# linnanwang/FastGen

Measured on AMD Instinct MI355X. Metric: images/sec at 4-step distilled (DMD2) sampling, higher is better.
Workload: dtype fp32 (tensors, accumulate) with split-bf16 x3 MFMA conv products; 1 GPU; EDM CIFAR-10 32x32 SongUNet (55.7M params) DMD2 4-step 'sde' sampling, batch=512 per GPU; global_batch=512, sample_steps=4, parallelism=replicas x1 (no data-path collective), graph=True

## Files before the change

fastgen_amd/csrc/attn.hip:

```cpp
#include <cstdlib>
#include "common.h"
#include "misc.h"

namespace {

template <typename T>
struct PFrag;
template <>
struct PFrag<__bf16> {
    static __device__ __forceinline__ Frag8<__bf16> make(const f32x16& p, int s) {
        Frag8<__bf16> f;
#pragma unroll
        for (int j = 0; j < 8; ++j) f.v[j] = (__bf16)p[8 * s + j];
        return f;
    }
};
template <>
struct PFrag<float> {
    static __device__ __forceinline__ Frag8<float> make(const f32x16& p, int s) {
        Frag8<float> f;
        f.lo = f32x4{p[8 * s + 0], p[8 * s + 1], p[8 * s + 2], p[8 * s + 3]};
        f.hi = f32x4{p[8 * s + 4], p[8 * s + 5], p[8 * s + 6], p[8 * s + 7]};
        return f;
    }
// ... 216 lines not shown
            sum += e;
        }
    sum += __shfl_xor(sum, 32);
    const float inv = __builtin_amdgcn_rcpf(sum);
    Frag8<__bf16> pf[8][2];
#pragma unroll
    for (int kt = 0; kt < 8; ++kt) {
#pragma unroll
        for (int s2 = 0; s2 < 2; ++s2)
#pragma unroll
            for (int j = 0; j < 8; ++j) pf[kt][s2].v[j] = (__bf16)(st[kt][8 * s2 + j] * inv);
        __builtin_amdgcn_sched_barrier(0);
    }

    __builtin_amdgcn_sched_barrier(0);
    __bf16* obase = out + ((size_t)n * Tn + q0) * D + r;
#pragma unroll 1
    for (int dg = 0; dg < 2; ++dg) {
        f32x16 o[4];
#pragma unroll
        for (int d = 0; d < 4; ++d)
#pragma unroll
            for (int i = 0; i < 16; ++i) o[d][i] = 0.f;
        asm volatile("" ::: "memory");
        stage_v(0, smem);
        __syncthreads();
#pragma unroll
        for (int t = 0; t < 4; ++t) {
            const char* cur = smem + (t & 1) * ATT_BUF;
            if (t + 1 < 4) stage_v(t + 1, smem + ((t + 1) & 1) * ATT_BUF);
#pragma unroll
            for (int sub = 0; sub < 2; ++sub)
#pragma unroll
                for (int s2 = 0; s2 < 2; ++s2)
#pragma unroll
                    for (int d = 0; d < 4; ++d) {
                        const char* p = cur + ((dg * 4 + d) * 32 + r) * VPITCH + (sub * 32 + 16 * s2 + 4 * h) * 2;
                        const bf16x4 lo = *reinterpret_cast<const bf16x4*>(p);
                        const bf16x4 hi = *reinterpret_cast<const bf16x4*>(p + 16);
                        Frag8<__bf16> vf;
                        vf.v = bf16x8{lo[0], lo[1], lo[2], lo[3], hi[0], hi[1], hi[2], hi[3]};
                        mma16(o[d], pf[t * 2 + sub][s2], vf);
                    }
            __syncthreads();
            __builtin_amdgcn_sched_barrier(0);
        }
#pragma unroll
        for (int d = 0; d < 4; ++d)
#pragma unroll
            for (int i = 0; i < 16; ++i) obase[(size_t)acc_row(i, h) * D + (dg * 4 + d) * 32] = (__bf16)o[d][i];
    }
}

constexpr int X3_KP = 272, X3_VP = 136;
constexpr int X3_PLANE = 64 * X3_KP;
constexpr int X3_BUF = 2 * X3_PLANE;

struct AttnMerge {
    const float2* ab;
    const float* bp;
    float2* stats;
    float scale;
};

template <bool MRG>
__global__ __launch_bounds__(256, 2) void attention_x3_lds_kernel(const float* __restrict__ q, const float* __restrict__ k,
                                                                  const float* __restrict__ vt, float* __restrict__ out, int B,
                                                                  AttnMerge mg) {
    constexpr int Tn = 256, D = 256;
    extern __shared__ __attribute__((aligned(16))) char smem[];
    const int tid = threadIdx.x, lane = tid & 63, wave = tid >> 6;
    const int r = lane & 31, h = lane >> 5;
    const int n = blockIdx.x >> 1;
    const int q0 = (blockIdx.x & 1) * 128 + wave * 32;

    auto stage_k = [&](int s, char* buf) {
        const float* src = k + ((size_t)n * Tn + (s & 3) * 64) * D + (s >> 2) * 128;
        f32x4 cf[4];
        if constexpr (MRG) {
            const f32x4* cp = reinterpret_cast<const f32x4*>(mg.ab + (size_t)n * D + (s >> 2) * 128 + (tid & 15) * 8);
#pragma unroll
            for (int j = 0; j < 4; ++j) cf[j] = cp[j];
        }
#pragma unroll
        for (int b2 = 0; b2 < 2; ++b2) {
#pragma unroll
            for (int i = b2 * 2; i < b2 * 2 + 2; ++i) {
                const int idx = tid + 256 * i, row = idx >> 4, c = idx & 15;
                float x[8];
                widen8(load_frag(src + (size_t)row * D + c * 8), x);
                if constexpr (MRG) {
#pragma unroll
                    for (int j = 0; j < 8; ++j) x[j] = fmaf(x[j], cf[j >> 1][2 * (j & 1)], cf[j >> 1][2 * (j & 1) + 1]);
                }
                bf16x8 hi, lo;
                split8(x, hi, lo);
                *reinterpret_cast<bf16x8*>(buf + row * X3_KP + c * 16) = hi;
                *reinterpret_cast<bf16x8*>(buf + X3_PLANE + row * X3_KP + c * 16) = lo;
            }
            __builtin_amdgcn_sched_barrier(0);
        }
    };
    auto stage_v = [&](int s, char* buf) {
        const float* src = vt + ((size_t)n * D + (s >> 2) * 128) * Tn + (s & 3) * 64;
#pragma unroll
        for (int b2 = 0; b2 < 2; ++b2) {
#pragma unroll
            for (int i = b2 * 2; i < b2 * 2 + 2; ++i) {
                const int idx = tid + 256 * i, row = idx >> 3, c = idx & 7;
                float x[8];
                widen8(load_frag(src + (size_t)row * Tn + c * 8), x);
                bf16x8 hi, lo;
                split8(x, hi, lo);
                bf16x4* dh = reinterpret_cast<bf16x4*>(buf + row * X3_VP + c * 16);
                dh[0] = bf16x4{hi[0], hi[1], hi[2], hi[3]};
                dh[1] = bf16x4{hi[4], hi[5], hi[6], hi[7]};
                bf16x4* dl = reinterpret_cast<bf16x4*>(buf + X3_PLANE + row * X3_VP + c * 16);
                dl[0] = bf16x4{lo[0], lo[1], lo[2], lo[3]};
                dl[1] = bf16x4{lo[4], lo[5], lo[6], lo[7]};
            }
            __builtin_amdgcn_sched_barrier(0);
        }
    };

    const float* qrow = q + ((size_t)n * Tn + q0 + r) * D + 8 * h;
    f32x16 st[8];
#pragma unroll
    for (int kt = 0; kt < 8; ++kt)
#pragma unroll
        for (int i = 0; i < 16; ++i) st[kt][i] = 0.f;

    stage_k(0, smem);
    __syncthreads();
    Frag8<bf16x3> qf[8];
#pragma unroll
    for (int s = 0; s < 8; ++s) {
        const char* cur = smem + (s & 1) * X3_BUF;
        if ((s & 3) == 0) {
#pragma unroll
            for (int kk = 0; kk < 8; ++kk) qf[kk] = load_op<bf16x3>(qrow + (s >> 2) * 128 + kk * 16);
        }
        if (s + 1 < 8) stage_k(s + 1, smem + ((s + 1) & 1) * X3_BUF);
#pragma unroll
        for (int kk = 0; kk < 8; ++kk) {
#pragma unroll
            for (int sub = 0; sub < 2; ++sub) {
                const char* p = cur + (sub * 32 + r) * X3_KP + (kk * 16 + 8 * h) * 2;
                Frag8<bf16x3> kf;
                kf.hi = *reinterpret_cast<const bf16x8*>(p);
                kf.lo = *reinterpret_cast<const bf16x8*>(p + X3_PLANE);
                mma16(st[(s & 3) * 2 + sub], kf, qf[kk]);
            }
        }
        __syncthreads();
        __builtin_amdgcn_sched_barrier(0);
    }

    float m = -INFINITY;
#pragma unroll
    for (int kt = 0; kt < 8; ++kt)
#pragma unroll
        for (int i = 0; i < 16; ++i) m = fmaxf(m, st[kt][i]);
    m = fmaxf(m, __shfl_xor(m, 32));
    float sum = 0.f;
#pragma unroll
    for (int kt = 0; kt < 8; ++kt)
#pragma unroll
        for (int i = 0; i < 16; ++i) {
            const float e = __builtin_amdgcn_exp2f(1.44269504088896341f * 0.0625f * (st[kt][i] - m));
            st[kt][i] = e;
            sum += e;
        }
    sum += __shfl_xor(sum, 32);
    const float inv = __builtin_amdgcn_rcpf(sum);
    Frag8<bf16x3> pf[8][2];
#pragma unroll
    for (int kt = 0; kt < 8; ++kt) {
#pragma unroll
        for (int s2 = 0; s2 < 2; ++s2) {
            float v[8];
#pragma unroll
            for (int j = 0; j < 8; ++j) v[j] = st[kt][8 * s2 + j] * inv;
            split8(v, pf[kt][s2].hi, pf[kt][s2].lo);
        }
        __builtin_amdgcn_sched_barrier(0);
    }

    float* obase = out + ((size_t)n * Tn + q0) * D + r;
    stage_v(0, smem);
    __syncthreads();
    f32x16 o[4];
#pragma unroll
    for (int s = 0; s < 8; ++s) {
        const char* cur = smem + (s & 1) * X3_BUF;
        if ((s & 3) == 0) {
#pragma unroll
            for (int d = 0; d < 4; ++d)
#pragma unroll
                for (int i = 0; i < 16; ++i) o[d][i] = 0.f;
        }
        if (s + 1 < 8) stage_v(s + 1, smem + ((s + 1) & 1) * X3_BUF);
#pragma unroll
        for (int sub = 0; sub < 2; ++sub)
#pragma unroll
            for (int s2 = 0; s2 < 2; ++s2)
#pragma unroll
                for (int d = 0; d < 4; ++d) {
                    const char* p = cur + (d * 32 + r) * X3_VP + (sub * 32 + 16 * s2 + 4 * h) * 2;
                    const bf16x4 a0 = *reinterpret_cast<const bf16x4*>(p), a1 = *reinterpret_cast<const bf16x4*>(p + 16);
                    const bf16x4 b0 = *reinterpret_cast<const bf16x4*>(p + X3_PLANE), b1 = *reinterpret_cast<const bf16x4*>(p + X3_PLANE + 16);
                    Frag8<bf16x3> vf;
                    vf.hi = bf16x8{a0[0], a0[1], a0[2], a0[3], a1[0], a1[1], a1[2], a1[3]};
                    vf.lo = bf16x8{b0[0], b0[1], b0[2], b0[3], b1[0], b1[1], b1[2], b1[3]};
                    mma16(o[d], pf[(s & 3) * 2 + sub][s2], vf);
                }
        __syncthreads();
        __builtin_amdgcn_sched_barrier(0);
        if ((s & 3) == 3) {
            if constexpr (MRG) {
                const float* xbase = k + ((size_t)n * Tn + q0) * D + r;
#pragma unroll
                for (int d = 0; d < 4; ++d) {
                    const int col = ((s >> 2) * 4 + d) * 32;
                    const float bias = mg.bp[col + r];
                    float sv = 0.f, qv = 0.f;
#pragma unroll
                    for (int i = 0; i < 16; ++i) {
                        const size_t off = (size_t)acc_row(i, h) * D + col;
                        const float v = (o[d][i] + bias + xbase[off]) * mg.scale;
                        obase[off] = v;
                        sv += v;
                        qv += v * v;
                    }
                    if (mg.stats) {
                        sv += __shfl_xor(sv, 32), qv += __shfl_xor(qv, 32);
                        sv += __shfl_xor(sv, 1), qv += __shfl_xor(qv, 1);
                        sv += __shfl_xor(sv, 2), qv += __shfl_xor(qv, 2);
                        if (h == 0 && (r & 3) == 0)
                            mg.stats[((size_t)n * 8 + (blockIdx.x & 1) * 4 + wave) * (D / 4) + ((col + r) >> 2)] = make_float2(sv, qv);
                    }
                }
            } else {
#pragma unroll
                for (int d = 0; d < 4; ++d)
#pragma unroll
                    for (int i = 0; i < 16; ++i) obase[(size_t)acc_row(i, h) * D + ((s >> 2) * 4 + d) * 32] = o[d][i];
            }
        }
    }
}

__global__ void attn_merge_weights_kernel(const float* __restrict__ qkv_w, const float* __restrict__ qkv_b, const float* __restrict__ proj_w,
                                          float* __restrict__ w_out, float* __restrict__ b_out, int C) {
    const int o = blockIdx.x % C;
    const bool val = blockIdx.x >= C;
    for (int i = threadIdx.x; i <= C; i += blockDim.x) {
        double acc = 0.0;
        for (int c = 0; c < C; ++c) {
            const double l = val ? proj_w[(size_t)o * C + c] : qkv_w[(size_t)(3 * c + 1) * C + o];
            const int row = 3 * c + (val ? 2 : 0);
            acc += l * (double)(i < C ? qkv_w[(size_t)row * C + i] : qkv_b[row]);
        }
        if (i < C)
            w_out[(size_t)blockIdx.x * C + i] = (float)acc;
        else
            b_out[blockIdx.x] = (float)acc;
    }
}

template <bool MRG>
int x3_lds_prepare() {
    static bool done[16] = {};
    const int dev = fg_device_slot();
    if (dev < 0) return (int)hipErrorInvalidDevice;
    if (!done[dev]) {
        hipError_t e = hipFuncSetAttribute(reinterpret_cast<const void*>(attention_x3_lds_kernel<MRG>), hipFuncAttributeMaxDynamicSharedMemorySize, 2 * X3_BUF);
        if (e != hipSuccess) return (int)e;
        done[dev] = true;
    }
    return 0;
}

}

int launch_attn_merge_weights(const float* qkv_w, const float* qkv_b, const float* proj_w, float* w_out, float* b_out, int C, hipStream_t s) {
    hipLaunchKernelGGL(attn_merge_weights_kernel, dim3(2 * C), dim3(256), 0, s, qkv_w, qkv_b, proj_w, w_out, b_out, C);
    return (int)hipGetLastError();
}

int launch_attention_merged(const float* qm, const float* x_mid, const float2* ab, const float* vmt, const float* bp, float scale, float* out,
                            float2* stats, int B, hipStream_t s) {
    const int rc = x3_lds_prepare<true>();
    if (rc || !qm) return rc;
    hipLaunchKernelGGL(attention_x3_lds_kernel<true>, dim3(B * 2), dim3(256), 2 * X3_BUF, s, qm, x_mid, vmt, out, B, AttnMerge{ab, bp, stats, scale});
    return (int)hipGetLastError();
}

int launch_attention(int dtype, const void* q, const void* k, const void* vt, void* out, int B, int T, hipStream_t s) {
    if (T != 256 && T != 64) return (int)hipErrorInvalidValue;
    const int nt = T / 32;
    const int waves = B * nt;
    dim3 grid((waves + 3) / 4), block(256);
    if (dtype == 1 && nt == 8) {
        static bool attr_done_dev[16] = {};
        const int dev = fg_device_slot();
        if (dev < 0) return (int)hipErrorInvalidDevice;
        bool& attr_done = attr_done_dev[dev];
        if (!attr_done) {
            hipError_t e = hipFuncSetAttribute(reinterpret_cast<const void*>(attention_lds_kernel), hipFuncAttributeMaxDynamicSharedMemorySize, 2 * ATT_BUF);
            if (e != hipSuccess) return (int)e;
            attr_done = true;
        }
        if (!q) return 0;
        hipLaunchKernelGGL(attention_lds_kernel, dim3(B * 2), block, 2 * ATT_BUF, s, (const __bf16*)q, (const __bf16*)k, (const __bf16*)vt, (__bf16*)out, B);
        return (int)hipGetLastError();
    }
    static const bool x3_lds = [] {
        const char* e = getenv("FASTGEN_AMD_ATTN_X3_LDS");
        return !(e && e[0] == '0');
    }();
    if (dtype == 2 && nt == 8 && x3_lds) {
        const int rc = x3_lds_prepare<false>();
        if (rc || !q) return rc;
        hipLaunchKernelGGL(attention_x3_lds_kernel<false>, dim3(B * 2), block, 2 * X3_BUF, s, (const float*)q, (const float*)k, (const float*)vt, (float*)out, B,
                           AttnMerge{});
        return (int)hipGetLastError();
    }
    if (!q) return 0;
    if (dtype == 2) {
        if (nt == 8)
            hipLaunchKernelGGL((attention_kernel<bf16x3, 8>), grid, block, 0, s, (const float*)q, (const float*)k, (const float*)vt, (float*)out, B);
        else
            hipLaunchKernelGGL((attention_kernel<bf16x3, 2>), grid, block, 0, s, (const float*)q, (const float*)k, (const float*)vt, (float*)out, B);
    } else if (dtype) {
        if (nt == 8)
            hipLaunchKernelGGL((attention_kernel<__bf16, 8>), grid, block, 0, s, (const __bf16*)q, (const __bf16*)k, (const __bf16*)vt, (__bf16*)out, B);
        else
            hipLaunchKernelGGL((attention_kernel<__bf16, 2>), grid, block, 0, s, (const __bf16*)q, (const __bf16*)k, (const __bf16*)vt, (__bf16*)out, B);
    } else {
        if (nt == 8)
            hipLaunchKernelGGL((attention_kernel<float, 8>), grid, block, 0, s, (const float*)q, (const float*)k, (const float*)vt, (float*)out, B);
        else
            hipLaunchKernelGGL((attention_kernel<float, 2>), grid, block, 0, s, (const float*)q, (const float*)k, (const float*)vt, (float*)out, B);
    }
    return (int)hipGetLastError();
}
```

fastgen_amd/csrc/engine.hip:

```cpp
#include <hip/hip_runtime.h>

#include <atomic>
#include <cmath>
#include <cstdarg>
#include <cstdio>
#include <cstdlib>
#include <cstring>
#include <string>
#include <map>
#include <vector>

#include "../../include/fastgen_amd.h"
#include "common.h"
#include "adm.h"
#include "edm2.h"
#include "conv.h"
#include "misc.h"

namespace {

thread_local std::string g_err;

int fail(int code, const char* fmt, ...) {
    char buf[512];
// ... 695 lines not shown
void use_stash(Workspace& w, const BlockStash& st) {
    w.h.p = st.h;
    w.ab0 = st.ab0, w.ab1 = st.ab1, w.mr0 = st.mr0, w.mr1 = st.mr1;
    w.a1d = st.a1d;
    w.drop.block = st.index;
    if (st.xattn) {
        w.xattn.p = st.xattn;
        w.ab2 = st.ab2, w.mr2 = st.mr2;
        w.q = st.q, w.k = st.k, w.vt = st.vt, w.aout = st.aout;
    }
}
int block_index(const fg_edm* h, const Block* b) {
    for (size_t i = 0; i < h->blocks.size(); ++i)
        if (h->blocks[i] == b) return (int)i;
    return -1;
}

bool attn_merge_enabled() {
    static const bool on = [] {
        const char* e = getenv("FASTGEN_AMD_ATTN_MERGE");
        return !(e && e[0] == '0');
    }();
    return on;
}

int run_block(fg_edm* h, const Block& b, const Act& x1, int c1, const Act& x2, int c2, const float* temb, Act& out, int B,
              Workspace& w, hipStream_t s) {
    if (c1 + c2 != b.cin) return fail(FG_EINVAL, "%s: got %d+%d input channels, expected %d", b.key.c_str(), c1, c2, b.cin);
    const int hw_in = b.res_in * b.res_in, hw = b.res_out * b.res_out;
    const int res_mode = b.down ? RES_DOWN : (b.up ? RES_UP : RES_NONE);
    const int slots = conv_stat_slots(b.res_out);
    int rc;
    if ((rc = norm_coeffs(h->dtype, x1, c1, x2, c2, h->P(b.norm0_w), h->P(b.norm0_b), w.ab0, B, hw_in, s, w.mr0))) return rc;
    ConvArgs a{};
    a.src1 = x1.p; a.src2 = c2 ? x2.p : nullptr; a.C1 = c1; a.C2 = c2;
    a.Hs = a.Ws = b.res_in; a.H = a.W = b.res_out; a.B = B;
    a.ab = w.ab0; a.wpack = b.p_conv0; a.wpack_ws = b.p_conv0_ws; a.bias = h->P(b.conv0_b);
    a.temb = temb + b.temb_off; a.temb_stride = h->temb_total;
    a.resid = nullptr; a.scale = 1.0f; a.out = w.h.p; a.Cout = b.cout; a.stats = w.h.st;
    const bool x3_up = b.up && w.infer && !w.a1d && h->cmode == FG_DTYPE_BF16X3 && conv_ws_enabled();
    bool sub0 = false;
    if (x3_up && conv_subpix_mode() == 2 && b.p_conv0_sub) {
        ConvArgs p = a;
        p.wpack_ws = b.p_conv0_sub;
        sub0 = conv_x3ws_supported(3, PRO_GN_SILU, RES_SUBPIX, OUT_NHWC, p);
    }
    if (sub0) {
        a.wpack_ws = b.p_conv0_sub;
        w.h.slots = conv_launch_stat_slots(h->cmode, 3, PRO_GN_SILU, RES_SUBPIX, OUT_NHWC, a);
        HIP_TRY(conv_launch(h, 3, PRO_GN_SILU, RES_SUBPIX, OUT_NHWC, a, s));
    } else if (b.down && !c2) {
        HIP_TRY(launch_gn_silu_pool(h->dtype, x1.p, w.ab0, w.pool, B, b.res_out, b.res_out, c1, s));
        a.src1 = w.pool; a.Hs = a.Ws = b.res_out; a.ab = nullptr;
        w.h.slots = conv_launch_stat_slots(h->cmode, 3, PRO_NONE, RES_NONE, OUT_NHWC, a);
        HIP_TRY(conv_launch(h, 3, PRO_NONE, RES_NONE, OUT_NHWC, a, s));
    } else {
        w.h.slots = conv_launch_stat_slots(h->cmode, 3, PRO_GN_SILU, res_mode, OUT_NHWC, a);
        HIP_TRY(conv_launch(h, 3, PRO_GN_SILU, res_mode, OUT_NHWC, a, s));
    }
    ConvArgs d{};
    d.src1 = w.h.p; d.C1 = b.cout; d.Hs = d.Ws = d.H = d.W = b.res_out; d.B = B;
    d.ab = w.ab1; d.wpack = b.p_conv1; d.wpack_ws = b.p_conv1_ws; d.bias = h->P(b.conv1_b);
    d.scale = kSkipScale; d.Cout = b.cout;
    const void* resid = x1.p;
    if (b.has_skip) {
        bool low = false;
        if (x3_up && conv_subpix_mode() >= 1) {
            ConvArgs p = d;
            p.resid = w.sbuf; p.rshift = 1;
            low = conv_x3ws_supported(3, PRO_GN_SILU, RES_NONE, OUT_NHWC, p);
        }
        ConvArgs k{};
        k.src1 = x1.p; k.src2 = c2 ? x2.p : nullptr; k.C1 = c1; k.C2 = c2;
        k.Hs = k.Ws = b.res_in; k.H = k.W = low ? b.res_in : b.res_out; k.B = B;
        k.wpack = b.p_skip; k.bias = h->P(b.skip_b); k.scale = 1.0f; k.out = w.sbuf; k.Cout = b.cout;
        HIP_TRY(conv_launch(h, 1, PRO_NONE, low ? RES_NONE : res_mode, OUT_NHWC, k, s));
        resid = w.sbuf;
        d.rshift = low ? 1 : 0;
    }
    HIP_TRY(launch_gn_finalize(w.h.st, b.cout, w.h.slots, nullptr, 0, 0, h->P(b.norm1_w), h->P(b.norm1_b), kBlockEps, w.ab1, B, hw, s, w.mr1));
    Act& x_mid = b.attn ? w.xattn : out;
    d.resid = resid; d.out = x_mid.p; d.stats = x_mid.st;
    if (w.a1d) {
        HIP_TRY(launch_gn_act(h->dtype, 0, w.h.p, b.cout, nullptr, 0, w.ab1, w.a1d, B, b.res_out, 0, s, w.drop));
        d.src1 = w.a1d; d.ab = nullptr;
        x_mid.slots = conv_launch_stat_slots(h->cmode, 3, PRO_NONE, RES_NONE, OUT_NHWC, d);
        HIP_TRY(conv_launch(h, 3, PRO_NONE, RES_NONE, OUT_NHWC, d, s));
    } else {
        x_mid.slots = conv_launch_stat_slots(h->cmode, 3, PRO_GN_SILU, RES_NONE, OUT_NHWC, d);
        HIP_TRY(conv_launch(h, 3, PRO_GN_SILU, RES_NONE, OUT_NHWC, d, s));
    }
    if (b.attn) {
        HIP_TRY(launch_gn_finalize(x_mid.st, b.cout, x_mid.slots, nullptr, 0, 0, h->P(b.norm2_w), h->P(b.norm2_b), kBlockEps, w.ab2, B, hw, s, w.mr2));
        ConvArgs q{};
        q.src1 = x_mid.p; q.C1 = b.cout; q.Hs = q.Ws = q.H = q.W = b.res_out; q.B = B;
        if (w.infer && !w.a1d && h->cmode == FG_DTYPE_BF16X3 && hw == 256 && b.cout == 256 && b.p_qv && attn_merge_enabled()) {
            q.ab = w.ab2; q.wpack = b.p_qv; q.bias = b.qv_bias; q.scale = 1.0f; q.Cout = 2 * b.cout;
            q.q_out = w.q; q.vt_out = w.vt;
            HIP_TRY(conv_launch(h, 1, PRO_GN, RES_NONE, OUT_QV, q, s));
            HIP_TRY(launch_attention_merged((const float*)w.q, (const float*)x_mid.p, w.ab2, (const float*)w.vt, h->P(b.proj_b), kSkipScale,
                                            (float*)out.p, out.st, B, s));
            out.slots = 8;
            return FG_OK;
        }
        q.ab = w.ab2; q.wpack = b.p_qkv; q.bias = b.qkv_bias; q.scale = 1.0f; q.Cout = 3 * b.cout;
        q.q_out = w.q; q.k_out = w.k; q.vt_out = w.vt;
// ... 54 lines not shown
                HIP_TRY(launch_act_to_nchw(h->dtype, w.skip[i].p, feats[b.tap], B, b.cout, b.res_out * b.res_out, s));
        }
        x = &w.skip[i];
    }
    if (early) return FG_OK;
    int sp = (int)h->enc.size();
    Act* pong[2] = {&w.xa, &w.xb};
    int cur = 0;
    size_t di = 0;
    const float2* aux_ab = nullptr;
    for (const Block& b : h->dec) {
        if (b.kind == K_BLOCK) {
            const Act& x2 = b.skip_c ? w.skip[--sp] : none;
            Act& dst = ts ? ts->dec_store[di++] : *pong[cur];
            if (ts) use_stash(w, ts->blocks[block_index(h, &b)]);
            rc = run_block(h, b, *x, b.cin - b.skip_c, x2, b.skip_c, w.temb, dst, B, w, s);
            if (rc) return rc;
            x = &dst;
            cur ^= 1;
        } else if (b.kind == K_AUX_NORM) {
            if (ts) w.ab0 = ts->aux_ab, w.mr0 = ts->aux_mr;
            if ((rc = norm_coeffs(h->dtype, *x, b.cin, none, 0, h->P(b.w), h->P(b.b), w.ab0, B, b.res_in * b.res_in, s, ts ? w.mr0 : nullptr))) return rc;
            aux_ab = w.ab0;
        } else if (b.kind == K_AUX_CONV) {
            if (b.p_aux)
                HIP_TRY(launch_aux_head(h->cmode, x->p, aux_ab, b.p_aux, h->P(b.b), x_t, w.coef, out, B, b.cin, b.cout, s, ts ? ts->raw_out : nullptr));
            else
                HIP_TRY(launch_aux_out(h->dtype, x->p, aux_ab, h->P(b.w), h->P(b.b), x_t, w.coef, out, B, b.res_out, b.cin, b.cout, s, ts ? ts->raw_out : nullptr));
        }
    }
    return FG_OK;
}

int enqueue_sampler(fg_edm* h, const float* noise, const float* labels, const double* t_list, int steps, int type,
                    int loop, const float* eps, float* out, int B, Workspace& w, hipStream_t s) {
    const fg_edm_config& c = h->cfg;
    const int64_t total = (int64_t)B * c.img_channels * c.img_resolution * c.img_resolution;
    const StudentLoop L{noise, t_list, steps, type, c.schedule, total, w.x, w.eps, eps, w.tl, w.seed, out, s};
    if (loop == FG_LOOP_MEANFLOW)
        return meanflow_loop(L, w.x_pred, [&](int i, float* u) {
            return run_forward(h, w.x, w.tl + i, 0, w.tl + (type == FG_SAMPLE_SDE ? steps : i + 1), 0, labels, u, B, w, s);
        });
    return x0_loop(L, w.x_pred, [&](int i, float* pred) { return run_forward(h, w.x, w.tl + i, 0, w.tl + steps, 0, labels, pred, B, w, s); });
}

int ensure_device_state(fg_edm* h) {
    if (h->device_ready) return FG_OK;
    int rc;
    const size_t tsz = h->dtype ? 2 : 4;
    for (Block* b : h->blocks) {
        if ((rc = h->alloc(&b->p_conv0, conv_pack_elems(b->cout, b->cin, 3) * tsz))) return rc;
        if ((rc = h->alloc(&b->p_conv1, conv_pack_elems(b->cout, b->cout, 3) * tsz))) return rc;
        const bool x3 = h->cmode == FG_DTYPE_BF16X3;
        if ((x3 ? conv_x3ws_shape_ok(b->cout, b->cin, b->res_out) : conv_ws_shape_ok(h->cmode, b->cout, b->cin, b->res_out)) && !b->down &&
            (rc = h->alloc(&b->p_conv0_ws, conv_pack_elems(b->cout, b->cin, 3) * tsz)))
            return rc;
        if ((x3 ? conv_x3ws_shape_ok(b->cout, b->cout, b->res_out) : conv_ws_shape_ok(h->cmode, b->cout, b->cout, b->res_out)) &&
            (rc = h->alloc(&b->p_conv1_ws, conv_pack_elems(b->cout, b->cout, 3) * tsz)))
            return rc;
        if (x3 && b->up && conv_x3ws_shape_ok(b->cout, b->cin, b->res_in) && (rc = h->alloc(&b->p_conv0_sub, conv_pack_elems(b->cout, b->cin, 4) * 4)))
            return rc;
        if (b->has_skip && (rc = h->alloc(&b->p_skip, conv_pack_elems(b->cout, b->cin, 1) * tsz))) return rc;
        if (b->attn) {
            if ((rc = h->alloc(&b->p_qkv, conv_pack_elems(3 * b->cout, b->cout, 1) * tsz))) return rc;
            if ((rc = h->alloc(&b->p_proj, conv_pack_elems(b->cout, b->cout, 1) * tsz))) return rc;
            if ((rc = h->alloc((void**)&b->qkv_bias, sizeof(float) * 3 * b->cout))) return rc;
            if (x3 && b->cout == 256 && b->res_out == 16) {
                if ((rc = h->alloc(&b->p_qv, conv_pack_elems(2 * b->cout, b->cout, 1) * tsz))) return rc;
                if ((rc = h->alloc((void**)&b->qv_bias, sizeof(float) * 2 * b->cout))) return rc;
                if (!h->qv_w && (rc = h->alloc((void**)&h->qv_w, sizeof(float) * 2 * b->cout * b->cout))) return rc;
            }
        }
    }
    for (Block& b : h->enc)
        if (b.kind == K_STEM && stem_supported(b.res_out, b.cin, b.cout))
            if ((rc = h->alloc(&b.p_stem, stem_pack_elems() * tsz))) return rc;
    for (Block& b : h->dec)
        if (b.kind == K_AUX_CONV && aux_head_supported(h->cmode, b.res_out, b.cin, b.cout))
            if ((rc = h->alloc(&b.p_aux, aux_pack_elems(b.cin) * tsz))) return rc;
    if ((rc = h->alloc((void**)&h->aff_w, sizeof(float) * (size_t)h->temb_total * h->emb_ch))) return rc;
    if ((rc = h->alloc((void**)&h->aff_b, sizeof(float) * (size_t)h->temb_total))) return rc;
    const int half = h->noise_ch / 2;
    std::vector<float> fr(half);
    for (int j = 0; j < half; ++j) fr[j] = powf(1.0f / 10000.0f, (float)j / (float)(half - 1));
    if ((rc = h->alloc((void**)&h->freqs, sizeof(float) * half))) return rc;
    HIP_TRY(hipMemcpy(h->freqs, fr.data(), sizeof(float) * half, hipMemcpyHostToDevice));
    if (conv_prepare_all(h->cmode) != 0) return fail(FG_EHIP, "hipFuncSetAttribute(dynamic LDS) failed");
    if (launch_attention(h->cmode, nullptr, nullptr, nullptr, nullptr, 1, 256, nullptr) != 0) return fail(FG_EHIP, "attention prepare failed");
    if (h->cmode == FG_DTYPE_BF16X3 && launch_attention_merged(nullptr, nullptr, nullptr, nullptr, nullptr, 0.f, nullptr, nullptr, 1, nullptr) != 0)
        return fail(FG_EHIP, "attention prepare failed");
    h->device_ready = true;
    return FG_OK;
}

#include "engine_adm.inc"

}

extern "C" {

const char* fg_last_error(void) { return g_err.c_str(); }
const char* fg_version(void) { return "fastgen_amd 0.1 gfx950"; }
void fg_graph_stats(uint64_t* captures, uint64_t* launches) {
    if (captures) *captures = g_graph_captures.load(std::memory_order_relaxed);
    if (launches) *launches = g_graph_launches.load(std::memory_order_relaxed);
}

// ... 852 lines not shown
```

fastgen_amd/csrc/engine_train.inc:

```

namespace {
struct BwdScratch {
    void *g1, *aop, *da, *dh0, *dskip, *dxin, *wpk, *wg;
    void *gmid = nullptr, *dq = nullptr, *dk = nullptr, *dvt = nullptr, *dqkv = nullptr, *att = nullptr;
    float2 *P, *S, *mr0, *mr1, *mr2;
    float *dtemb, *wt;
    size_t wg_bytes;
};
int pad256(int c) { return (c + 255) / 256 * 256; }
size_t block_wgrad_bytes(int B, int res, int cin, int cout, bool attn) {
    size_t m = 0;
    const int shapes[5][3] = {{cout, cout, 3}, {cin, cout, 3}, {cin, cout, 1}, {cout, 3 * cout, 1}, {cout, cout, 1}};
    for (int i = 0; i < (attn ? 5 : 3); ++i)
        if (conv_wgrad_supported(res, shapes[i][0], shapes[i][1], shapes[i][2]))
            m = std::max(m, conv_wgrad_workspace_bytes(B, res, shapes[i][0], shapes[i][1], shapes[i][2]));
    return m;
}
size_t plan_block_bwd(const fg_edm* h, int B, int res_in, int res, int cin, int cout, Arena& A, BwdScratch& q, int attn_hw = 0, size_t wg_bytes = 0) {
    const size_t tsz = h->dtype ? 2 : 4, wsz = h->cmode == FG_DTYPE_BF16 ? 2 : 4;
    const size_t npix = (size_t)B * res * res, npix_in = (size_t)B * res_in * res_in;
    const int cp = pad256(cin), cm = cin > cout ? cin : cout;
    q.g1 = A.take(npix * cout * tsz);
    q.aop = A.take(npix * cm * tsz);
    q.da = A.take(npix * (cp > cout ? cp : cout) * tsz);
// ... 393 lines not shown
        HIP_TRY(launch_linear(w.emb1, h->P(w1), h->P(b1), nb.pre, B, E, E, 0, s));
        HIP_TRY(launch_silu_bwd(nb.demb, nb.pre, nb.d1, B * E, s));
        HIP_TRY(hipMemsetAsync(nb.d0, 0, sizeof(float) * (size_t)B * E, s));
        HIP_TRY(launch_linear_bwd(nb.d1, w.emb1, h->P(w1), h->G(w1), h->G(b1), nb.d0, B, E, E, 1.0f, s));
        HIP_TRY(launch_linear(w.emb0, h->P(w0), h->P(b0), nb.pre, B, N, E, 0, s));
        HIP_TRY(launch_silu_bwd(nb.d0, nb.pre, nb.d1, B * E, s));
        HIP_TRY(hipMemsetAsync(nb.d0, 0, sizeof(float) * (size_t)B * N, s));
        HIP_TRY(launch_linear_bwd(nb.d1, w.emb0, h->P(w0), h->G(w0), h->G(b0), nb.d0, B, E, N, 1.0f, s));
        if (h->augment && c.augment_dim > 0) {
            const int wa = h->find("model.map_augment.weight");
            if (h->G(wa)) HIP_TRY(launch_linear_bwd(nb.d0, h->augment, nullptr, h->G(wa), nullptr, nullptr, B, N, c.augment_dim, 1.0f, s));
        }
        if (c.label_dim > 0) {
            const int wl = h->find("model.map_label.weight"), bl = h->find("model.map_label.bias");
            HIP_TRY(launch_linear_bwd(nb.d0, labels, nullptr, labels ? h->G(wl) : nullptr, h->G(bl), nullptr, B, N, c.label_dim,
                                      std::sqrt((float)c.label_dim), s));
        }
    }
    return FG_OK;
}

int tangent_conv(fg_edm* h, int ks, int res_mode, const void* src, int cin, int res_in, int res_out, const void* wpack, int cout,
                 const float* temb, const void* resid, float scale, void* out, int B, hipStream_t s, const void* wpack_ws = nullptr) {
    ConvArgs a{};
    a.src1 = src; a.C1 = cin; a.C2 = 0;
    a.Hs = a.Ws = res_in; a.H = a.W = res_out; a.B = B;
    a.wpack = wpack; a.wpack_ws = wpack_ws; a.bias = nullptr;
    a.temb = temb; a.temb_stride = h->temb_total;
    a.resid = resid; a.scale = scale; a.out = out; a.Cout = cout;
    HIP_TRY(launch_conv_fused(h->cmode, ks, PRO_NONE, res_mode, OUT_NHWC, a, s));
    return FG_OK;
}

int block_jvp(fg_edm* h, const Block& b, const Act& a1, int c1, const void* xd1, const Act& a2, int c2, const void* xd2,
              const float* dtemb, void* yd, int B, Workspace& w, BwdScratch& q, const BlockStash& st, const float2* ident_ab,
              hipStream_t s) {
    const int res = b.res_out, res_in = b.res_in, hw = res * res, cin = b.cin, cout = b.cout;
    const int rm = b.down ? 1 : (b.up ? 2 : 0);
    const int res_mode = b.down ? RES_DOWN : (b.up ? RES_UP : RES_NONE);
    int rc;
    use_stash(w, st);
    const void* xd = xd1;
    if (c2) {
        HIP_TRY(launch_gn_act(h->dtype, 2, xd1, c1, xd2, c2, nullptr, q.aop, B, res_in, 0, s));
        xd = q.aop;
    }
    HIP_TRY(launch_gn_jvp(h->dtype, 0, a1.p, c1, c2 ? a2.p : nullptr, c2, xd, st.ab0, st.mr0, q.P, q.S, q.da, B, res_in, s));
    const void* ad0 = q.da;
    if (rm) {
        HIP_TRY(launch_gn_act(h->dtype, 2, q.da, cin, nullptr, 0, nullptr, q.dskip, B, res, rm, s));
        ad0 = q.dskip;
    }
    if ((rc = tangent_conv(h, 3, RES_NONE, ad0, cin, res, res, b.p_conv0, cout, dtemb + b.temb_off, nullptr, 1.0f, q.dh0, B, s,
                           b.p_conv0_ws))) return rc;
    DropArgs drop;
    if (st.a1d && h->dropout_p > 0.f) drop.p = h->dropout_p, drop.seed = h->dropout_seed, drop.block = st.index;
    HIP_TRY(launch_gn_jvp(h->dtype, 0, st.h, cout, nullptr, 0, q.dh0, st.ab1, st.mr1, q.P, q.S, q.g1, B, res, s, drop));
    const void* sd = xd;
    if (b.has_skip) {
        if ((rc = tangent_conv(h, 1, res_mode, xd, cin, res_in, res, b.p_skip, cout, nullptr, nullptr, 1.0f, q.dxin, B, s))) return rc;
        sd = q.dxin;
    }
    void* mid = b.attn ? q.gmid : yd;
    if ((rc = tangent_conv(h, 3, RES_NONE, q.g1, cout, res, res, b.p_conv1, cout, nullptr, sd, kSkipScale, mid, B, s, b.p_conv1_ws))) return rc;
    if (b.attn) {
        HIP_TRY(launch_gn_jvp(h->dtype, 1, st.xattn, cout, nullptr, 0, q.gmid, st.ab2, st.mr2, q.P, q.S, q.da, B, res, s));
        ConvArgs qa{};
        qa.src1 = q.da; qa.C1 = cout; qa.Hs = qa.Ws = qa.H = qa.W = res; qa.B = B;
        qa.ab = ident_ab; qa.wpack = b.p_qkv; qa.bias = nullptr; qa.scale = 1.0f; qa.Cout = 3 * cout;
        qa.q_out = q.dq; qa.k_out = q.dk; qa.vt_out = q.dvt;
        HIP_TRY(launch_conv_fused(h->cmode, 1, PRO_GN, RES_NONE, OUT_QKV, qa, s));
        HIP_TRY(launch_attention_jvp(h->dtype, st.q, st.k, st.vt, q.dq, q.dk, q.dvt, q.da, q.att, B, hw, cout, s));
        if ((rc = tangent_conv(h, 1, RES_NONE, q.da, cout, res, res, b.p_proj, cout, nullptr, q.gmid, kSkipScale, yd, B, s))) return rc;
    }
    return FG_OK;
}

int run_jvp(fg_edm* h, const float* x_t, const double* t, const double* r, const float* labels, const float* vx, const float* vt,
            const float* vr, float* out, float* jvp, int B, Workspace& w, NetBwd& nb, hipStream_t s) {
    const fg_edm_config& c = h->cfg;
    const int res = c.img_resolution, hw = res * res, C = c.img_channels;
    BwdScratch& q = nb.q;
    if (h->dropout_p <= 0.f)
        for (BlockStash& st : nb.ts.blocks) st.a1d = nullptr;
    int rc = run_forward(h, x_t, t, 1, r, 1, labels, out, B, w, s, nullptr, false, &nb.ts);
    if (rc) return rc;
    const Block *aux_norm = nullptr, *aux_conv = nullptr;
    for (const Block& b : h->dec) {
        if (b.kind == K_AUX_NORM) aux_norm = &b;
        if (b.kind == K_AUX_CONV) aux_conv = &b;
    }
    if (!aux_norm || !aux_conv || aux_conv->cin != 256 || !h->enc[0].p_stem || !q.att)
        return fail(FG_EINVAL, "jvp: head / stem shape not covered");
    const int E = h->emb_ch, N = h->cond_ch, TT = h->temb_total;
    float* ct = nb.vec_all;
    if (8 * B > TT) return fail(FG_EINVAL, "jvp: batch too large for the coefficient scratch");
    float* e0 = nb.d0;
    float* dtemb = nb.dtemb_all;
    float2* ident = (float2*)nb.pre;
    float* ones = nb.vec;
    float* zeros = nb.vec + 512;
    if (B > 512) return fail(FG_EINVAL, "jvp: batch too large for the constant scratch");
    HIP_TRY(launch_fill_f32(ones, 1.0f, 512, s));
    HIP_TRY(launch_fill_f32(zeros, 0.0f, 512, s));
    HIP_TRY(launch_jvp_coef(t, c.r_timestep ? r : nullptr, vt, vr, c.sigma_data, h->shift(), c.drop_precond, ct, B, s));
    {
        const int w1 = h->find("model.map_layer1.weight"), b1 = h->find("model.map_layer1.bias");
// ... 195 lines not shown
```

Baseline: 2915 img/s.

## Merge attention query halves into one 512-thread block and overlap K/V staging

The x3 attention kernel now runs one 512-thread block per image instead of two 256-thread blocks, so every K/V tile staged in LDS is shared by all 256 queries rather than loaded and split twice. Staging is split into a global load issued before the MFMA loop and an LDS commit after it, so load latency overlaps compute. The V LDS layout is changed so each fragment is read with a single bf16x8 load, at the cost of a larger plane. Separately, the engine allows the x3 weight-stationary conv pack for downsampling conv0 in inference only. This costs occupancy (launch bounds drop to one block per CU) and extra registers for the held loads.

Result: no change. 2926 img/s (median of 6 runs) (+0.4%).

```diff
diff --git a/fastgen_amd/csrc/attn.hip b/fastgen_amd/csrc/attn.hip
--- a/fastgen_amd/csrc/attn.hip
+++ b/fastgen_amd/csrc/attn.hip
@@ -292,9 +292,10 @@
     }
 }
 
-constexpr int X3_KP = 272, X3_VP = 136;
-constexpr int X3_PLANE = 64 * X3_KP;
+constexpr int X3_KP = 272, X3_VP = 144;
+constexpr int X3_PLANE = 128 * X3_VP;
 constexpr int X3_BUF = 2 * X3_PLANE;
+constexpr int X3_THREADS = 512;
 
 struct AttnMerge {
     const float2* ab;
@@ -304,62 +305,71 @@
 };
 
 template <bool MRG>
-__global__ __launch_bounds__(256, 2) void attention_x3_lds_kernel(const float* __restrict__ q, const float* __restrict__ k,
-                                                                  const float* __restrict__ vt, float* __restrict__ out, int B,
-                                                                  AttnMerge mg) {
+__global__ __launch_bounds__(X3_THREADS, 1) void attention_x3_lds_kernel(const float* __restrict__ q, const float* __restrict__ k,
+                                                                         const float* __restrict__ vt, float* __restrict__ out, int B,
+                                                                         AttnMerge mg) {
     constexpr int Tn = 256, D = 256;
     extern __shared__ __attribute__((aligned(16))) char smem[];
     const int tid = threadIdx.x, lane = tid & 63, wave = tid >> 6;
     const int r = lane & 31, h = lane >> 5;
-    const int n = blockIdx.x >> 1;
-    const int q0 = (blockIdx.x & 1) * 128 + wave * 32;
-
-    auto stage_k = [&](int s, char* buf) {
+    const int n = blockIdx.x;
+    const int q0 = wave * 32;
+
+    Frag8<float> held[2];
+    f32x4 cf[4];
+    auto load_k = [&](int s) {
         const float* src = k + ((size_t)n * Tn + (s & 3) * 64) * D + (s >> 2) * 128;
-        f32x4 cf[4];
         if constexpr (MRG) {
-            const f32x4* cp = reinterpret_cast<const f32x4*>(mg.ab + (size_t)n * D + (s >> 2) * 128 + (tid & 15) * 8);
-#pragma unroll
-            for (int j = 0; j < 4; ++j) cf[j] = cp[j];
-        }
-#pragma unroll
-        for (int b2 = 0; b2 < 2; ++b2) {
-#pragma unroll
-            for (int i = b2 * 2; i < b2 * 2 + 2; ++i) {
-                const int idx = tid + 256 * i, row = idx >> 4, c = idx & 15;
-                float x[8];
-                widen8(load_frag(src + (size_t)row * D + c * 8), x);
-                if constexpr (MRG) {
-#pragma unroll
-                    for (int j = 0; j < 8; ++j) x[j] = fmaf(x[j], cf[j >> 1][2 * (j & 1)], cf[j >> 1][2 * (j & 1) + 1]);
-                }
-                bf16x8 hi, lo;
-                split8(x, hi, lo);
-                *reinterpret_cast<bf16x8*>(buf + row * X3_KP + c * 16) = hi;
-                *reinterpret_cast<bf16x8*>(buf + X3_PLANE + row * X3_KP + c * 16) = lo;
-            }
-            __builtin_amdgcn_sched_barrier(0);
+            if ((s & 3) == 0) {
+                const f32x4* cp = reinterpret_cast<const f32x4*>(mg.ab + (size_t)n * D + (s >> 2) * 128 + (tid & 15) * 8);
+#pragma unroll
+                for (int j = 0; j < 4; ++j) cf[j] = cp[j];
+            }
+        }
+#pragma unroll
+        for (int i = 0; i < 2; ++i) {
+            const int idx = tid + X3_THREADS * i, row = idx >> 4, c = idx & 15;
+            held[i] = load_frag(src + (size_t)row * D + c * 8);
         }
     };
-    auto stage_v = [&](int s, char* buf) {
+    auto commit_k = [&](char* buf) {
+#pragma unroll
+        for (int i = 0; i < 2; ++i) {
+            const int idx = tid + X3_THREADS * i, row = idx >> 4, c = idx & 15;
+            float x[8];
+            widen8(held[i], x);
+            if constexpr (MRG) {
+#pragma unroll
+                for (int j = 0; j < 8; ++j) x[j] = fmaf(x[j], cf[j >> 1][2 * (j & 1)], cf[j >> 1][2 * (j & 1) + 1]);
+            }
+            bf16x8 hi, lo;
+            split8(x, hi, lo);
+            *reinterpret_cast<bf16x8*>(buf + row * X3_KP + c * 16) = hi;
+            *reinterpret_cast<bf16x8*>(buf + X3_PLANE + row * X3_KP + c * 16) = lo;
+        }
+    };
+    auto load_v = [&](int s) {
         const float* src = vt + ((size_t)n * D + (s >> 2) * 128) * Tn + (s & 3) * 64;
 #pragma unroll
-        for (int b2 = 0; b2 < 2; ++b2) {
-#pragma unroll
-            for (int i = b2 * 2; i < b2 * 2 + 2; ++i) {
-                const int idx = tid + 256 * i, row = idx >> 3, c = idx & 7;
-                float x[8];
-                widen8(load_frag(src + (size_t)row * Tn + c * 8), x);
-                bf16x8 hi, lo;
-                split8(x, hi, lo);
-                bf16x4* dh = reinterpret_cast<bf16x4*>(buf + row * X3_VP + c * 16);
-                dh[0] = bf16x4{hi[0], hi[1], hi[2], hi[3]};
-                dh[1] = bf16x4{hi[4], hi[5], hi[6], hi[7]};
-                bf16x4* dl = reinterpret_cast<bf16x4*>(buf + X3_PLANE + row * X3_VP + c * 16);
-                dl[0] = bf16x4{lo[0], lo[1], lo[2], lo[3]};
-                dl[1] = bf16x4{lo[4], lo[5], lo[6], lo[7]};
-            }
-            __builtin_amdgcn_sched_barrier(0);
+        for (int i = 0; i < 2; ++i) {
+            const int idx = tid + X3_THREADS * i, row = idx >> 3, c = idx & 7;
+            held[i] = load_frag(src + (size_t)row * Tn + c * 8);
+        }
+    };
+    auto commit_v = [&](char* buf) {
+#pragma unroll
+        for (int i = 0; i < 2; ++i) {
+            const int idx = tid + X3_THREADS * i, row = idx >> 3, c = idx & 7;
+            float x[8];
+            widen8(held[i], x);
+            bf16x8 hi, lo;
+            split8(x, hi, lo);
+            bf16x4* dh = reinterpret_cast<bf16x4*>(buf + row * X3_VP + (c >> 1) * 32 + (c & 1) * 8);
+            dh[0] = bf16x4{hi[0], hi[1], hi[2], hi[3]};
+            dh[2] = bf16x4{hi[4], hi[5], hi[6], hi[7]};
+            bf16x4* dl = reinterpret_cast<bf16x4*>(buf + X3_PLANE + row * X3_VP + (c >> 1) * 32 + (c & 1) * 8);
+            dl[0] = bf16x4{lo[0], lo[1], lo[2], lo[3]};
+            dl[2] = bf16x4{lo[4], lo[5], lo[6], lo[7]};
         }
     };
 
@@ -370,7 +380,8 @@
 #pragma unroll
         for (int i = 0; i < 16; ++i) st[kt][i] = 0.f;
 
-    stage_k(0, smem);
+    load_k(0);
+    commit_k(smem);
     __syncthreads();
     Frag8<bf16x3> qf[8];
 #pragma unroll
@@ -380,7 +391,8 @@
 #pragma unroll
             for (int kk = 0; kk < 8; ++kk) qf[kk] = load_op<bf16x3>(qrow + (s >> 2) * 128 + kk * 16);
         }
-        if (s + 1 < 8) stage_k(s + 1, smem + ((s + 1) & 1) * X3_BUF);
+        if (s + 1 < 8) load_k(s + 1);
+        __builtin_amdgcn_sched_barrier(0);
 #pragma unroll
         for (int kk = 0; kk < 8; ++kk) {
 #pragma unroll
@@ -392,6 +404,8 @@
                 mma16(st[(s & 3) * 2 + sub], kf, qf[kk]);
             }
         }
+        __builtin_amdgcn_sched_barrier(0);
+        if (s + 1 < 8) commit_k(smem + ((s + 1) & 1) * X3_BUF);
         __syncthreads();
         __builtin_amdgcn_sched_barrier(0);
     }
@@ -427,7 +441,8 @@
     }
 
     float* obase = out + ((size_t)n * Tn + q0) * D + r;
-    stage_v(0, smem);
+    load_v(0);
+    commit_v(smem);
     __syncthreads();
     f32x16 o[4];
 #pragma unroll
@@ -439,21 +454,22 @@
 #pragma unroll
                 for (int i = 0; i < 16; ++i) o[d][i] = 0.f;
         }
-        if (s + 1 < 8) stage_v(s + 1, smem + ((s + 1) & 1) * X3_BUF);
+        if (s + 1 < 8) load_v(s + 1);
+        __builtin_amdgcn_sched_barrier(0);
 #pragma unroll
         for (int sub = 0; sub < 2; ++sub)
 #pragma unroll
             for (int s2 = 0; s2 < 2; ++s2)
 #pragma unroll
                 for (int d = 0; d < 4; ++d) {
-                    const char* p = cur + (d * 32 + r) * X3_VP + (sub * 32 + 16 * s2 + 4 * h) * 2;
-                    const bf16x4 a0 = *reinterpret_cast<const bf16x4*>(p), a1 = *reinterpret_cast<const bf16x4*>(p + 16);
-                    const bf16x4 b0 = *reinterpret_cast<const bf16x4*>(p + X3_PLANE), b1 = *reinterpret_cast<const bf16x4*>(p + X3_PLANE + 16);
+                    const char* p = cur + (d * 32 + r) * X3_VP + (sub * 2 + s2) * 32 + h * 16;
                     Frag8<bf16x3> vf;
-                    vf.hi = bf16x8{a0[0], a0[1], a0[2], a0[3], a1[0], a1[1], a1[2], a1[3]};
-                    vf.lo = bf16x8{b0[0], b0[1], b0[2], b0[3], b1[0], b1[1], b1[2], b1[3]};
+                    vf.hi = *reinterpret_cast<const bf16x8*>(p);
+                    vf.lo = *reinterpret_cast<const bf16x8*>(p + X3_PLANE);
                     mma16(o[d], pf[(s & 3) * 2 + sub][s2], vf);
                 }
+        __builtin_amdgcn_sched_barrier(0);
+        if (s + 1 < 8) commit_v(smem + ((s + 1) & 1) * X3_BUF);
         __syncthreads();
         __builtin_amdgcn_sched_barrier(0);
         if ((s & 3) == 3) {
@@ -477,7 +493,7 @@
                         sv += __shfl_xor(sv, 1), qv += __shfl_xor(qv, 1);
                         sv += __shfl_xor(sv, 2), qv += __shfl_xor(qv, 2);
                         if (h == 0 && (r & 3) == 0)
-                            mg.stats[((size_t)n * 8 + (blockIdx.x & 1) * 4 + wave) * (D / 4) + ((col + r) >> 2)] = make_float2(sv, qv);
+                            mg.stats[((size_t)n * 8 + wave) * (D / 4) + ((col + r) >> 2)] = make_float2(sv, qv);
                     }
                 }
             } else {
@@ -532,7 +548,7 @@
                             float2* stats, int B, hipStream_t s) {
     const int rc = x3_lds_prepare<true>();
     if (rc || !qm) return rc;
-    hipLaunchKernelGGL(attention_x3_lds_kernel<true>, dim3(B * 2), dim3(256), 2 * X3_BUF, s, qm, x_mid, vmt, out, B, AttnMerge{ab, bp, stats, scale});
+    hipLaunchKernelGGL(attention_x3_lds_kernel<true>, dim3(B), dim3(X3_THREADS), 2 * X3_BUF, s, qm, x_mid, vmt, out, B, AttnMerge{ab, bp, stats, scale});
     return (int)hipGetLastError();
 }
 
@@ -562,7 +578,7 @@
     if (dtype == 2 && nt == 8 && x3_lds) {
         const int rc = x3_lds_prepare<false>();
         if (rc || !q) return rc;
-        hipLaunchKernelGGL(attention_x3_lds_kernel<false>, dim3(B * 2), block, 2 * X3_BUF, s, (const float*)q, (const float*)k, (const float*)vt, (float*)out, B,
+        hipLaunchKernelGGL(attention_x3_lds_kernel<false>, dim3(B), dim3(X3_THREADS), 2 * X3_BUF, s, (const float*)q, (const float*)k, (const float*)vt, (float*)out, B,
                            AttnMerge{});
         return (int)hipGetLastError();
     }
diff --git a/fastgen_amd/csrc/engine.hip b/fastgen_amd/csrc/engine.hip
--- a/fastgen_amd/csrc/engine.hip
+++ b/fastgen_amd/csrc/engine.hip
@@ -771,6 +771,7 @@
     } else if (b.down && !c2) {
         HIP_TRY(launch_gn_silu_pool(h->dtype, x1.p, w.ab0, w.pool, B, b.res_out, b.res_out, c1, s));
         a.src1 = w.pool; a.Hs = a.Ws = b.res_out; a.ab = nullptr;
+        if (!w.infer || w.a1d) a.wpack_ws = nullptr;
         w.h.slots = conv_launch_stat_slots(h->cmode, 3, PRO_NONE, RES_NONE, OUT_NHWC, a);
         HIP_TRY(conv_launch(h, 3, PRO_NONE, RES_NONE, OUT_NHWC, a, s));
     } else {
@@ -931,7 +932,7 @@
         if ((rc = h->alloc(&b->p_conv0, conv_pack_elems(b->cout, b->cin, 3) * tsz))) return rc;
         if ((rc = h->alloc(&b->p_conv1, conv_pack_elems(b->cout, b->cout, 3) * tsz))) return rc;
         const bool x3 = h->cmode == FG_DTYPE_BF16X3;
-        if ((x3 ? conv_x3ws_shape_ok(b->cout, b->cin, b->res_out) : conv_ws_shape_ok(h->cmode, b->cout, b->cin, b->res_out)) && !b->down &&
+        if ((x3 ? conv_x3ws_shape_ok(b->cout, b->cin, b->res_out) : conv_ws_shape_ok(h->cmode, b->cout, b->cin, b->res_out) && !b->down) &&
             (rc = h->alloc(&b->p_conv0_ws, conv_pack_elems(b->cout, b->cin, 3) * tsz)))
             return rc;
         if ((x3 ? conv_x3ws_shape_ok(b->cout, b->cout, b->res_out) : conv_ws_shape_ok(h->cmode, b->cout, b->cout, b->res_out)) &&
diff --git a/fastgen_amd/csrc/engine_train.inc b/fastgen_amd/csrc/engine_train.inc
--- a/fastgen_amd/csrc/engine_train.inc
+++ b/fastgen_amd/csrc/engine_train.inc
@@ -469,7 +469,7 @@
         ad0 = q.dskip;
     }
     if ((rc = tangent_conv(h, 3, RES_NONE, ad0, cin, res, res, b.p_conv0, cout, dtemb + b.temb_off, nullptr, 1.0f, q.dh0, B, s,
-                           b.p_conv0_ws))) return rc;
+                           b.down ? nullptr : b.p_conv0_ws))) return rc;
     DropArgs drop;
     if (st.a1d && h->dropout_p > 0.f) drop.p = h->dropout_p, drop.seed = h->dropout_seed, drop.block = st.index;
     HIP_TRY(launch_gn_jvp(h->dtype, 0, st.h, cout, nullptr, 0, q.dh0, st.ab1, st.mr1, q.P, q.S, q.g1, B, res, s, drop));
```

## Warp-specialize x3 attention with producer waves and triple-buffered LDS staging

Applied to the files above, without the earlier changes.

Grows the x3 attention block to 512 threads. Four producer waves load the K and V tiles from global memory, apply the merge affine, split each value into bf16 hi/lo and store it into a three-slot LDS ring. The four consumer waves only issue MFMAs and step in lockstep through a lightweight lgkmcnt+s_barrier, and the second Q half is prefetched during the K loop. The goal is to overlap global loads and conversion with the matrix math. In exchange LDS use grows from two to three buffers and occupancy drops, since launch_bounds no longer requests two blocks per CU. The barrier counts between producer and consumer must match exactly.

After: 2886 img/s before, 2882 img/s after. No clear change (-0.2%).

```diff
diff --git a/fastgen_amd/csrc/attn.hip b/fastgen_amd/csrc/attn.hip
--- a/fastgen_amd/csrc/attn.hip
+++ b/fastgen_amd/csrc/attn.hip
@@ -295,6 +295,13 @@
 constexpr int X3_KP = 272, X3_VP = 136;
 constexpr int X3_PLANE = 64 * X3_KP;
 constexpr int X3_BUF = 2 * X3_PLANE;
+constexpr int X3_SLOTS = 3;
+constexpr int X3_LDS = X3_SLOTS * X3_BUF;
+constexpr int X3_ATT_NTHR = 512;
+
+__device__ __forceinline__ void x3_step_barrier() {
+    asm volatile("s_waitcnt lgkmcnt(0)\n\ts_barrier" ::: "memory");
+}
 
 struct AttnMerge {
     const float2* ab;
@@ -304,65 +311,91 @@
 };
 
 template <bool MRG>
-__global__ __launch_bounds__(256, 2) void attention_x3_lds_kernel(const float* __restrict__ q, const float* __restrict__ k,
-                                                                  const float* __restrict__ vt, float* __restrict__ out, int B,
-                                                                  AttnMerge mg) {
+__global__ __launch_bounds__(X3_ATT_NTHR) void attention_x3_lds_kernel(const float* __restrict__ q, const float* __restrict__ k,
+                                                                       const float* __restrict__ vt, float* __restrict__ out, int B,
+                                                                       AttnMerge mg) {
     constexpr int Tn = 256, D = 256;
     extern __shared__ __attribute__((aligned(16))) char smem[];
     const int tid = threadIdx.x, lane = tid & 63, wave = tid >> 6;
     const int r = lane & 31, h = lane >> 5;
     const int n = blockIdx.x >> 1;
+
+    if (wave >= 4) {
+        const int pt = tid - 256;
+        float x[2][4][8];
+        f32x4 cf[2][4];
+        auto load_tile = [&](int t, float (&xs)[4][8]) {
+            if (t < 8) {
+                const float* src = k + ((size_t)n * Tn + (t & 3) * 64) * D + (t >> 2) * 128;
+#pragma unroll
+                for (int i = 0; i < 4; ++i) {
+                    const int idx = pt + 256 * i, row = idx >> 4, c = idx & 15;
+                    widen8(load_frag(src + (size_t)row * D + c * 8), xs[i]);
+                }
+            } else {
+                const float* src = vt + ((size_t)n * D + ((t - 8) >> 2) * 128) * Tn + (t & 3) * 64;
+#pragma unroll
+                for (int i = 0; i < 4; ++i) {
+                    const int idx = pt + 256 * i, row = idx >> 3, c = idx & 7;
+                    widen8(load_frag(src + (size_t)row * Tn + c * 8), xs[i]);
+                }
+            }
+        };
+        auto load_cf = [&](int half) {
+            if constexpr (MRG) {
+                const f32x4* cp = reinterpret_cast<const f32x4*>(mg.ab + (size_t)n * D + half * 128 + (pt & 15) * 8);
+#pragma unroll
+                for (int j = 0; j < 4; ++j) cf[half][j] = cp[j];
+            }
+        };
+        auto store_tile = [&](int t, float (&xs)[4][8], char* buf) {
+            if (t < 8) {
+#pragma unroll
+                for (int i = 0; i < 4; ++i) {
+                    const int idx = pt + 256 * i, row = idx >> 4, c = idx & 15;
+                    if constexpr (MRG) {
+#pragma unroll
+                        for (int j = 0; j < 8; ++j) xs[i][j] = fmaf(xs[i][j], cf[t >> 2][j >> 1][2 * (j & 1)], cf[t >> 2][j >> 1][2 * (j & 1) + 1]);
+                    }
+                    bf16x8 hi, lo;
+                    split8(xs[i], hi, lo);
+                    *reinterpret_cast<bf16x8*>(buf + row * X3_KP + c * 16) = hi;
+                    *reinterpret_cast<bf16x8*>(buf + X3_PLANE + row * X3_KP + c * 16) = lo;
+                }
+            } else {
+#pragma unroll
+                for (int i = 0; i < 4; ++i) {
+                    const int idx = pt + 256 * i, row = idx >> 3, c = idx & 7;
+                    bf16x8 hi, lo;
+                    split8(xs[i], hi, lo);
+                    bf16x4* dh = reinterpret_cast<bf16x4*>(buf + row * X3_VP + c * 16);
+                    dh[0] = bf16x4{hi[0], hi[1], hi[2], hi[3]};
+                    dh[1] = bf16x4{hi[4], hi[5], hi[6], hi[7]};
+                    bf16x4* dl = reinterpret_cast<bf16x4*>(buf + X3_PLANE + row * X3_VP + c * 16);
+                    dl[0] = bf16x4{lo[0], lo[1], lo[2], lo[3]};
+                    dl[1] = bf16x4{lo[4], lo[5], lo[6], lo[7]};
+                }
+            }
+        };
+
+        load_cf(0);
+        load_tile(0, x[0]);
+        load_tile(1, x[1]);
+        __builtin_amdgcn_sched_barrier(0);
+        store_tile(0, x[0], smem);
+        x3_step_barrier();
+#pragma unroll
+        for (int s = 0; s < 15; ++s) {
+            if (s + 2 < 16) load_tile(s + 2, x[s & 1]);
+            if (s + 2 == 4) load_cf(1);
+            __builtin_amdgcn_sched_barrier(0);
+            store_tile(s + 1, x[(s + 1) & 1], smem + ((s + 1) % X3_SLOTS) * X3_BUF);
+            x3_step_barrier();
+        }
+        return;
+    }
+
     const int q0 = (blockIdx.x & 1) * 128 + wave * 32;
-
-    auto stage_k = [&](int s, char* buf) {
-        const float* src = k + ((size_t)n * Tn + (s & 3) * 64) * D + (s >> 2) * 128;
-        f32x4 cf[4];
-        if constexpr (MRG) {
-            const f32x4* cp = reinterpret_cast<const f32x4*>(mg.ab + (size_t)n * D + (s >> 2) * 128 + (tid & 15) * 8);
-#pragma unroll
-            for (int j = 0; j < 4; ++j) cf[j] = cp[j];
-        }
-#pragma unroll
-        for (int b2 = 0; b2 < 2; ++b2) {
-#pragma unroll
-            for (int i = b2 * 2; i < b2 * 2 + 2; ++i) {
-                const int idx = tid + 256 * i, row = idx >> 4, c = idx & 15;
-                float x[8];
-                widen8(load_frag(src + (size_t)row * D + c * 8), x);
-                if constexpr (MRG) {
-#pragma unroll
-                    for (int j = 0; j < 8; ++j) x[j] = fmaf(x[j], cf[j >> 1][2 * (j & 1)], cf[j >> 1][2 * (j & 1) + 1]);
-                }
-                bf16x8 hi, lo;
-                split8(x, hi, lo);
-                *reinterpret_cast<bf16x8*>(buf + row * X3_KP + c * 16) = hi;
-                *reinterpret_cast<bf16x8*>(buf + X3_PLANE + row * X3_KP + c * 16) = lo;
-            }
-            __builtin_amdgcn_sched_barrier(0);
-        }
-    };
-    auto stage_v = [&](int s, char* buf) {
-        const float* src = vt + ((size_t)n * D + (s >> 2) * 128) * Tn + (s & 3) * 64;
-#pragma unroll
-        for (int b2 = 0; b2 < 2; ++b2) {
-#pragma unroll
-            for (int i = b2 * 2; i < b2 * 2 + 2; ++i) {
-                const int idx = tid + 256 * i, row = idx >> 3, c = idx & 7;
-                float x[8];
-                widen8(load_frag(src + (size_t)row * Tn + c * 8), x);
-                bf16x8 hi, lo;
-                split8(x, hi, lo);
-                bf16x4* dh = reinterpret_cast<bf16x4*>(buf + row * X3_VP + c * 16);
-                dh[0] = bf16x4{hi[0], hi[1], hi[2], hi[3]};
-                dh[1] = bf16x4{hi[4], hi[5], hi[6], hi[7]};
-                bf16x4* dl = reinterpret_cast<bf16x4*>(buf + X3_PLANE + row * X3_VP + c * 16);
-                dl[0] = bf16x4{lo[0], lo[1], lo[2], lo[3]};
-                dl[1] = bf16x4{lo[4], lo[5], lo[6], lo[7]};
-            }
-            __builtin_amdgcn_sched_barrier(0);
-        }
-    };
-
     const float* qrow = q + ((size_t)n * Tn + q0 + r) * D + 8 * h;
     f32x16 st[8];
 #pragma unroll
@@ -370,29 +403,37 @@
 #pragma unroll
         for (int i = 0; i < 16; ++i) st[kt][i] = 0.f;
 
-    stage_k(0, smem);
-    __syncthreads();
     Frag8<bf16x3> qf[8];
+    Frag8<float> qraw[8];
+#pragma unroll
+    for (int kk = 0; kk < 8; ++kk) qf[kk] = load_op<bf16x3>(qrow + kk * 16);
+    x3_step_barrier();
 #pragma unroll
     for (int s = 0; s < 8; ++s) {
-        const char* cur = smem + (s & 1) * X3_BUF;
-        if ((s & 3) == 0) {
-#pragma unroll
-            for (int kk = 0; kk < 8; ++kk) qf[kk] = load_op<bf16x3>(qrow + (s >> 2) * 128 + kk * 16);
-        }
-        if (s + 1 < 8) stage_k(s + 1, smem + ((s + 1) & 1) * X3_BUF);
+        int lofs = r * X3_KP + h * 16;
+        asm volatile("" : "+v"(lofs));
+        const char* cur = smem + (s % X3_SLOTS) * X3_BUF + lofs;
+        if (s == 4) {
+#pragma unroll
+            for (int kk = 0; kk < 8; ++kk) {
+                float v[8];
+                widen8(qraw[kk], v);
+                split8(v, qf[kk].hi, qf[kk].lo);
+            }
+        }
 #pragma unroll
         for (int kk = 0; kk < 8; ++kk) {
 #pragma unroll
             for (int sub = 0; sub < 2; ++sub) {
-                const char* p = cur + (sub * 32 + r) * X3_KP + (kk * 16 + 8 * h) * 2;
+                const char* p = cur + sub * 32 * X3_KP + kk * 32;
                 Frag8<bf16x3> kf;
                 kf.hi = *reinterpret_cast<const bf16x8*>(p);
                 kf.lo = *reinterpret_cast<const bf16x8*>(p + X3_PLANE);
                 mma16(st[(s & 3) * 2 + sub], kf, qf[kk]);
             }
-        }
-        __syncthreads();
+            if (s == 3) qraw[kk] = load_frag(qrow + 128 + kk * 16);
+        }
+        x3_step_barrier();
         __builtin_amdgcn_sched_barrier(0);
     }
 
@@ -427,26 +468,25 @@
     }
 
     float* obase = out + ((size_t)n * Tn + q0) * D + r;
-    stage_v(0, smem);
-    __syncthreads();
     f32x16 o[4];
 #pragma unroll
     for (int s = 0; s < 8; ++s) {
-        const char* cur = smem + (s & 1) * X3_BUF;
+        int lofs = r * X3_VP + h * 8;
+        asm volatile("" : "+v"(lofs));
+        const char* cur = smem + ((8 + s) % X3_SLOTS) * X3_BUF + lofs;
         if ((s & 3) == 0) {
 #pragma unroll
             for (int d = 0; d < 4; ++d)
 #pragma unroll
                 for (int i = 0; i < 16; ++i) o[d][i] = 0.f;
         }
-        if (s + 1 < 8) stage_v(s + 1, smem + ((s + 1) & 1) * X3_BUF);
 #pragma unroll
         for (int sub = 0; sub < 2; ++sub)
 #pragma unroll
             for (int s2 = 0; s2 < 2; ++s2)
 #pragma unroll
                 for (int d = 0; d < 4; ++d) {
-                    const char* p = cur + (d * 32 + r) * X3_VP + (sub * 32 + 16 * s2 + 4 * h) * 2;
+                    const char* p = cur + d * 32 * X3_VP + (sub * 32 + 16 * s2) * 2;
                     const bf16x4 a0 = *reinterpret_cast<const bf16x4*>(p), a1 = *reinterpret_cast<const bf16x4*>(p + 16);
                     const bf16x4 b0 = *reinterpret_cast<const bf16x4*>(p + X3_PLANE), b1 = *reinterpret_cast<const bf16x4*>(p + X3_PLANE + 16);
                     Frag8<bf16x3> vf;
@@ -454,7 +494,7 @@
                     vf.lo = bf16x8{b0[0], b0[1], b0[2], b0[3], b1[0], b1[1], b1[2], b1[3]};
                     mma16(o[d], pf[(s & 3) * 2 + sub][s2], vf);
                 }
-        __syncthreads();
+        if (s < 7) x3_step_barrier();
         __builtin_amdgcn_sched_barrier(0);
         if ((s & 3) == 3) {
             if constexpr (MRG) {
@@ -514,7 +554,7 @@
     const int dev = fg_device_slot();
     if (dev < 0) return (int)hipErrorInvalidDevice;
     if (!done[dev]) {
-        hipError_t e = hipFuncSetAttribute(reinterpret_cast<const void*>(attention_x3_lds_kernel<MRG>), hipFuncAttributeMaxDynamicSharedMemorySize, 2 * X3_BUF);
+        hipError_t e = hipFuncSetAttribute(reinterpret_cast<const void*>(attention_x3_lds_kernel<MRG>), hipFuncAttributeMaxDynamicSharedMemorySize, X3_LDS);
         if (e != hipSuccess) return (int)e;
         done[dev] = true;
     }
@@ -532,7 +572,7 @@
                             float2* stats, int B, hipStream_t s) {
     const int rc = x3_lds_prepare<true>();
     if (rc || !qm) return rc;
-    hipLaunchKernelGGL(attention_x3_lds_kernel<true>, dim3(B * 2), dim3(256), 2 * X3_BUF, s, qm, x_mid, vmt, out, B, AttnMerge{ab, bp, stats, scale});
+    hipLaunchKernelGGL(attention_x3_lds_kernel<true>, dim3(B * 2), dim3(X3_ATT_NTHR), X3_LDS, s, qm, x_mid, vmt, out, B, AttnMerge{ab, bp, stats, scale});
     return (int)hipGetLastError();
 }
 
@@ -562,7 +602,7 @@
     if (dtype == 2 && nt == 8 && x3_lds) {
         const int rc = x3_lds_prepare<false>();
         if (rc || !q) return rc;
-        hipLaunchKernelGGL(attention_x3_lds_kernel<false>, dim3(B * 2), block, 2 * X3_BUF, s, (const float*)q, (const float*)k, (const float*)vt, (float*)out, B,
+        hipLaunchKernelGGL(attention_x3_lds_kernel<false>, dim3(B * 2), dim3(X3_ATT_NTHR), X3_LDS, s, (const float*)q, (const float*)k, (const float*)vt, (float*)out, B,
                            AttnMerge{});
         return (int)hipGetLastError();
     }
```
